# qq456cvb/CanonicalVoting

Hardware: AMD Instinct MI355X
Metric: scenes/sec (80k-pt synthetic scans) (higher is better)
Workload: dtype f32

## Files before the change

### canonicalvoting_amd/csrc/cv_common.h

```cpp
#pragma once
#include <hip/hip_runtime.h>

#include <cstdarg>
#include <cstdint>
#include <cstdio>

#include "cv_hip.h"

void cv_set_error(const char* fmt, ...);

#define CV_HIP_CHECK(expr)                                                                  \
    do {                                                                                    \
        hipError_t e_ = (expr);                                                             \
        if (e_ != hipSuccess) {                                                             \
            cv_set_error("%s failed: %s (%s:%d)", #expr, hipGetErrorString(e_), __FILE__,   \
                         __LINE__);                                                         \
            return CV_EHIP;                                                                 \
        }                                                                                   \
    } while (0)

#define CV_LAUNCH_CHECK() CV_HIP_CHECK(hipGetLastError())

#define CV_REQUIRE(cond, code, ...)     \
    do {                                \
        if (!(cond)) {                  \
            cv_set_error(__VA_ARGS__);  \
            return (code);              \
        }                               \
    } while (0)

__host__ __device__ static inline size_t cv_align_up(size_t v, size_t a) { return (v + a - 1) / a * a; }

struct CvCarver {
    char* base;
    size_t off = 0;
    explicit CvCarver(void* p) : base(static_cast<char*>(p)) {}
    template <typename T>
    T* take(size_t count) {
        off = cv_align_up(off, 256);
        T* r = reinterpret_cast<T*>(base + off);
        off += count * sizeof(T);
        return r;
    }
};

struct CvMapJob {
    const int32_t* out_coords; long long n_out;
    const unsigned long long* keys; const int32_t* vals; long long cap;
    int k, ts;
    int32_t* nbr;
    const int32_t* compose;
    const unsigned* bitmap;
    const int32_t* bbox;
    int up;
    int32_t* nbr3;
    int32_t* mask_words;
};
constexpr int CV_MAX_MAP_JOBS = 12;
int cv_sp_kernel_maps_batch(const CvMapJob* jobs, int n_jobs, void* stream);
constexpr long long CV_BITMAP_WORDS = 1ll << 20;
int cv_sp_occupancy_bitmap(const int32_t* d_coords, long long n, const int32_t* d_bbox, unsigned* d_bits, void* stream,
                           bool pre_cleared = false);

int cv_sp_build_levels_zero(int32_t* const* d_coords, unsigned long long* const* d_keys, int32_t* const* d_vals,
                            long long n, long long cap, int num_levels, int32_t* d_counts, int32_t* h_counts, void* d_ws,
                            size_t ws_bytes, int32_t* d_zero, long long n_zero, int32_t* d_set_one, void* stream,
                            uint32_t* d_bits = nullptr);

struct CvUpJob { const int32_t* nbr_down; long long n_coarse; int32_t* up; };
int cv_sp_up_maps_batch(const CvUpJob* jobs, int n_jobs, void* stream);

struct CvPermJob {
    const int32_t* nbr; long long n; int K, groups; int32_t* perm; int with_map;
    const int32_t* mask_words;
};
constexpr int CV_MAX_PERM_JOBS = 8;
int cv_hv_minmax_async_ex(const float* d_points, int64_t n, float* h_minmax6, void* d_ws, size_t ws_bytes, int32_t* d_zero_word,
                          int32_t* d_fill7f, void* stream);
int cv_decode_f32_ev(float* d_grid_obj, const float* d_grid_rot, const float* d_grid_scale, const int dims[3],
                     const float h_corner3[3], float res, const float* d_points, const float* d_xyz, const float* d_prob,
                     const int32_t* d_class, int64_t n, const cv_decode_params* params, int mutate_grid, void* d_ws, size_t ws_bytes,
                     int* h_n_cand, int64_t* h_cand_idx, int32_t* h_verdict, int* h_n_boxes, float* h_boxes, float* h_scores,
                     int32_t* h_classes, int* h_truncated, void* stream, void* ev_done);
int cv_decode_cat_f32_ev(float* d_grid_obj, const float* d_grid_rot, const float* d_grid_scale, const int dims[3],
                         const float h_corner3[3], float res, const float* d_points, const float* d_xyz, const float* d_prob,
                         const int32_t* d_class, int64_t n, int num_cats, const cv_decode_params* params, int mutate_grid,
                         void* d_ws, size_t ws_bytes, int* h_n_cand, int64_t* h_cand_idx, int32_t* h_verdict, int* h_n_boxes,
                         float* h_boxes, float* h_scores, int32_t* h_classes, int* h_truncated, void* stream, void* ev_done);
int cv_sp_sort_rows_ex(const int32_t* d_coords, long long n, int32_t* d_sorted, int32_t* d_perm, int32_t* d_inv, void* d_ws,
                       size_t ws_bytes, bool single_batch, void* stream, bool bounds_prefilled = false);
int cv_sp_scene_plan_ex(const int32_t* d_input, long long n, int32_t* d_perm, int32_t* d_inv, int32_t* const* d_coords,
                        unsigned long long* const* d_keys, int32_t* const* d_vals, long long cap, int32_t* d_counts,
                        int32_t* h_counts, int stem_k, int mask_groups, long long masked_min_rows,
                        int32_t* d_arena, size_t arena_words, cv_scene_maps* offsets, void* d_sort_ws, size_t sort_ws_bytes,
                        void* d_levels_ws, size_t levels_ws_bytes, bool single_batch, void* stream,
                        bool bounds_prefilled = false);
int cv_sp_mask_perms_batch(const CvPermJob* jobs, int n_jobs, void* d_ws, size_t ws_bytes, void* stream,
                           bool pre_zeroed = false);
```

### canonicalvoting_amd/csrc/hv_decode.hip

```cpp
#include "cv_common.h"

#include <cmath>
#include <cstring>
#include <mutex>
#include <vector>

namespace {

#ifndef DEC_PROF
#define DEC_PROF 0
#endif
constexpr int NCLS = 64;

struct Cand {
    long long idx;
    int c[3];
    int clo[3], chi[3];
    float cw[3];
    float cs, sn;
    float sc[3];
};

struct Stats {
    unsigned n_in, n_mask, pmax_bits, pad;
// ... 37 lines not shown
}

__global__ __launch_bounds__(256) void dec_compact(const float* __restrict__ g_obj,
                                                   const float* __restrict__ g_rot,
                                                   const float* __restrict__ g_scale, Geo geo,
                                                   int64_t G, float thresh, List L,
                                                   unsigned* __restrict__ list_n, CatStride ks) {
    const int kc = blockIdx.y;
    g_obj = g_obj + kc * ks.cells; g_rot = g_rot + kc * 2 * ks.cells; g_scale = g_scale + kc * 3 * ks.cells;
    L = cat_list(L, ks.ws, kc); list_n = cat_ws(list_n, ks.ws, kc);
    for (int64_t base = blockIdx.x * 256ll; base < G; base += (int64_t)gridDim.x * 256) {
        const int64_t i = base + threadIdx.x;
        float v = 0.f;
        bool hit = false;
        if (i < G) { v = g_obj[i]; hit = v >= thresh; }
        const uint64_t m = __ballot(hit);
        if (m == 0) continue;
        unsigned pos = 0;
        const int lane = threadIdx.x & 63;
        const int leader = __ffsll((unsigned long long)m) - 1;
        if (lane == leader) pos = atomicAdd(list_n, (unsigned)__popcll(m));
        pos = __shfl(pos, leader);
        if (hit) {
            const unsigned p = pos + lanes_below(m);
            const int id = (int)i;
            L.idx[p] = id;
            L.val[p] = v;
            const int z = id % geo.Z, y = (id / geo.Z) % geo.Y, x = id / (geo.Z * geo.Y);
            L.xy[p] = (unsigned)x | ((unsigned)y << 16);
            L.z[p] = z;
            const float r0 = g_rot[(int64_t)id * 2], r1 = g_rot[(int64_t)id * 2 + 1];
            const float rot = (float)atan2((double)r1, (double)r0);
            L.geo[0 * L.cap + p] = (float)cos((double)rot);
            L.geo[1 * L.cap + p] = (float)sin((double)rot);
            for (int k = 0; k < 3; ++k) L.geo[(2 + k) * L.cap + p] = g_scale[(int64_t)id * 3 + k];
        }
    }
}

__device__ __forceinline__ bool inv_coords(float d0, float d1, float d2, float c, float s,
                                           const float* sc, float& w0, float& w1, float& w2) {
    w0 = fmaf(d2, s, fmaf(d1, 0.f, d0 * c)) / sc[0];
    w1 = fmaf(d2, 0.f, fmaf(d1, 1.f, d0 * 0.f)) / sc[1];
    w2 = fmaf(d2, c, fmaf(d1, 0.f, d0 * (-s))) / sc[2];
    return -1 < w0 && w0 < 1 && -1 < w1 && w1 < 1 && -1 < w2 && w2 < 1;
}

__device__ __forceinline__ bool inside_box(float d0, float d1, float d2, float c, float s, const float* sc) {
    const float t0 = fmaf(d2, s, fmaf(d1, 0.f, d0 * c));
    const float t1 = fmaf(d2, 0.f, fmaf(d1, 1.f, d0 * 0.f));
    const float t2 = fmaf(d2, c, fmaf(d1, 0.f, d0 * (-s)));
    return fabsf(t0) < fabsf(sc[0]) && fabsf(t1) < fabsf(sc[1]) && fabsf(t2) < fabsf(sc[2]);
}

__device__ __forceinline__ void box_corners(float cs, float sn, const float* sc, float* bb) {
    constexpr float kRawX[8] = {1, 1, -1, -1, 1, 1, -1, -1};
    constexpr float kRawY[8] = {1, 1, 1, 1, -1, -1, -1, -1};
    constexpr float kRawZ[8] = {1, -1, -1, 1, 1, -1, -1, 1};
    const float m00 = cs * sc[0], m02 = (-sn) * sc[2], m11 = sc[1], m20 = sn * sc[0], m22 = cs * sc[2];
#pragma unroll
    for (int q = 0; q < 8; ++q) {
        bb[q * 3 + 0] = m00 * kRawX[q] + m02 * kRawZ[q];
        bb[q * 3 + 1] = m11 * kRawY[q];
        bb[q * 3 + 2] = m20 * kRawX[q] + m22 * kRawZ[q];
    }
}

struct Best {
    float v;
    int id, pos;
};

__device__ __forceinline__ void take_better(Best& b, float v, int id, int pos) {
    if (v > b.v || (v == b.v && id < b.id)) { b.v = v; b.id = id; b.pos = pos; }
}

#ifndef DEC_SMALL_T
#define DEC_SMALL_T 512
#endif
constexpr int GREEDY_T = DEC_SMALL_T;
constexpr int GREEDY_W = GREEDY_T / 64;
constexpr int GREEDY_CAP = 4096;

template <int CTRL>
__device__ __forceinline__ int dpp_mov(int x) {
    return __builtin_amdgcn_update_dpp(x, x, CTRL, 0xf, 0xf, false);
}
__device__ __forceinline__ float wave_max_f32(float x) {
    x = fmaxf(x, __int_as_float(dpp_mov<0xB1>(__float_as_int(x))));
    x = fmaxf(x, __int_as_float(dpp_mov<0x4E>(__float_as_int(x))));
    x = fmaxf(x, __int_as_float(dpp_mov<0x124>(__float_as_int(x))));
    x = fmaxf(x, __int_as_float(dpp_mov<0x128>(__float_as_int(x))));
    const int xi = __float_as_int(x);
    const float a = __int_as_float(__builtin_amdgcn_readlane(xi, 0)), b = __int_as_float(__builtin_amdgcn_readlane(xi, 16)),
                c = __int_as_float(__builtin_amdgcn_readlane(xi, 32)), d = __int_as_float(__builtin_amdgcn_readlane(xi, 48));
    return fmaxf(fmaxf(a, b), fmaxf(c, d));
}
__device__ __forceinline__ int wave_min_i32(int x) {
    x = min(x, dpp_mov<0xB1>(x));
    x = min(x, dpp_mov<0x4E>(x));
    x = min(x, dpp_mov<0x124>(x));
    x = min(x, dpp_mov<0x128>(x));
    return min(min(__builtin_amdgcn_readlane(x, 0), __builtin_amdgcn_readlane(x, 16)),
               min(__builtin_amdgcn_readlane(x, 32), __builtin_amdgcn_readlane(x, 48)));
}

template <int MODE, int T>
__device__ __forceinline__ void dec_greedy(Geo geo, cv_decode_params prm, List L,
                                           const unsigned* __restrict__ list_n, Cand* __restrict__ cands,
                                           Stats* __restrict__ stats, int* __restrict__ n_cand_out) {
    constexpr bool IN_REG = MODE != 0, IN_LDS = MODE == 1;
    constexpr int GREEDY_E = (MODE == 1 ? GREEDY_CAP / T : 16);
    constexpr int CAP = IN_LDS ? GREEDY_E * T : 1;
    constexpr int GREEDY_T = T, GREEDY_W = T / 64;
    __shared__ unsigned l_xy[CAP];
    __shared__ int l_z[CAP];
    __shared__ float l_geo[5][CAP];
    __shared__ float s_val[2][GREEDY_W];
    __shared__ int s_idx[2][GREEDY_W], s_pos[2][GREEDY_W];
    const int n = (int)*list_n;
    float r_val[GREEDY_E];
    unsigned r_xy[GREEDY_E], dead = 0;
    int r_z[GREEDY_E], r_id[GREEDY_E];
    if (IN_REG) {
#pragma unroll
        for (int j = 0; j < GREEDY_E; ++j) {
            const int k = (int)threadIdx.x + j * GREEDY_T;
            const bool ok = k < n;
            r_val[j] = ok ? L.val[k] : 0.f;
            r_xy[j] = ok ? L.xy[k] : 0u;
            r_z[j] = ok ? L.z[k] : 0;
            r_id[j] = ((int)(r_xy[j] & 0xffffu) * geo.Y + (int)(r_xy[j] >> 16)) * geo.Z + r_z[j];
            dead |= ok ? 0u : (1u << j);
            if (ok && IN_LDS) {
                l_xy[k] = r_xy[j];
                l_z[k] = r_z[j];
                for (int q = 0; q < 5; ++q) l_geo[q][k] = L.geo[q * L.cap + k];
            }
        }
        __syncthreads();
    }
    const int wave = threadIdx.x >> 6;
    const float inv_res = 1.0f / geo.res;
    const int e = prm.elimination, hp = e + (prm.elim_hi_plus1 ? 1 : 0);
    bool have_cur = false;
    int cx = 0, cy = 0, cz = 0, clo0 = 0, clo1 = 0, clo2 = 0, chi0 = 0, chi1 = 0, chi2 = 0;
    int rlo0 = 0, rlo1 = 0, rlo2 = 0;
    unsigned rsp0 = 0, rsp1 = 0, rsp2 = 0;
    float ccs = 0.f, csn = 0.f, csc[3] = {1.f, 1.f, 1.f};
    auto flat_id = [&](int pos) {
        const unsigned xy = L.xy[pos];
        const int z = L.z[pos];
        return ((int)(xy & 0xffffu) * geo.Y + (int)(xy >> 16)) * geo.Z + z;
    };
    int it = 0;
    bool truncated = false;
    for (;; ++it) {
        float bv = -1.f;
        int bpos = -1, bid = 0x7fffffff;
        if constexpr (IN_REG) {
            if (have_cur) {
                unsigned near = 0;
#pragma unroll
                for (int j = 0; j < GREEDY_E; ++j) {
                    const int x = (int)(r_xy[j] & 0xffffu), y = (int)(r_xy[j] >> 16), z = r_z[j];
                    const bool in = (unsigned)(x - rlo0) <= rsp0 && (unsigned)(y - rlo1) <= rsp1 &&
                                    (unsigned)(z - rlo2) <= rsp2;
                    near |= in ? (1u << j) : 0u;
                }
                near &= ~dead;
// ... 730 lines not shown
```

### canonicalvoting_amd/csrc/sparse_conv.hip

```cpp
#include "cv_common.h"

#include <atomic>
#include <cstring>
#include <type_traits>
#include <utility>

#include "sparse_conv_common.h"

using namespace cvsc;

namespace {

template <int NB, bool VEC>
__global__ __launch_bounds__(THREADS) void conv_rows(ConvArgs a) {
    __shared__ float A_s[KC][A_LD];
    __shared__ float B_s[KC][NB * 32];
    __shared__ int nbr_s[TM];
    __shared__ int rows_s[TM];
    __shared__ __attribute__((aligned(16))) float ep_s[4][32][EP_LD];
    const int tid = threadIdx.x, lane = tid & 63, wave = tid >> 6;
    const int n0 = blockIdx.y * (NB * 32);

    if (tid < TM) {
        const long long tile_id = a.row_perm ? (long long)gridDim.x - 1 - blockIdx.x : blockIdx.x;
// ... 383 lines not shown
                             : make_float4(0.f, 0.f, 0.f, 0.f);
        }
        const unsigned short* slab = second ? a.wp6_2 + (long long)c * P * a.cout * 32
                                            : a.wp6 + (long long)(j * nch + c) * P * a.cout * 32;
#pragma unroll
        for (int i = 0; i < B_PER; ++i) {
            const int f = tid + i * THREADS;
            if (f < B_U4) {
                const int p = f / (NB * 32 * 4), rem = f - p * (NB * 32 * 4);
                const int col = rem >> 2, ch = rem & 3;
                rb[i] = (n0 + col < a.cout)
                            ? *reinterpret_cast<const uint4*>(slab + ((long long)p * a.cout + n0 + col) * 32 + ch * 8)
                            : make_uint4(0u, 0u, 0u, 0u);
            }
        }
    };
    auto stage = [&](unsigned char* Bb) {
#pragma unroll
        for (int i = 0; i < 4; ++i) {
            const int r = a_row + 8 * i;
            unsigned h0 = 0, m0 = 0, l0 = 0, h1 = 0, m1 = 0, l1 = 0;
            unsigned char* dst = A_h + r * 64 + ((((a_col >> 3) ^ ((r >> 2) & 3))) << 4) + ((a_col & 7) << 1);
            if constexpr (P == 1) {
                *reinterpret_cast<uint2*>(dst) = make_uint2(cvt_pk_bf16(ra[i].x, ra[i].y), cvt_pk_bf16(ra[i].z, ra[i].w));
            } else if constexpr (P == 3) {
                split3(ra[i].x, ra[i].y, h0, m0, l0);
                split3(ra[i].z, ra[i].w, h1, m1, l1);
                *reinterpret_cast<uint2*>(dst) = make_uint2(h0, h1);
                *reinterpret_cast<uint2*>(dst + TM * 64) = make_uint2(m0, m1);
                *reinterpret_cast<uint2*>(dst + 2 * TM * 64) = make_uint2(l0, l1);
            } else {
                in_max = fmaxf(fmaxf(in_max, fmaxf(fabsf(ra[i].x), fabsf(ra[i].y))), fmaxf(fabsf(ra[i].z), fabsf(ra[i].w)));
                split2h(ra[i].x, ra[i].y, h0, l0);
                split2h(ra[i].z, ra[i].w, h1, l1);
                *reinterpret_cast<uint2*>(dst) = make_uint2(h0, h1);
                *reinterpret_cast<uint2*>(dst + TM * 64) = make_uint2(l0, l1);
            }
        }
#pragma unroll
        for (int i = 0; i < B_PER; ++i) {
            const int f = tid + i * THREADS;
            if (f < B_U4) {
                const int p = f / (NB * 32 * 4), rem = f - p * (NB * 32 * 4);
                const int col = rem >> 2, ch = rem & 3;
                *reinterpret_cast<uint4*>(Bb + (p * NB * 32 + col) * 64 + ((ch ^ ((col >> 2) & 3)) << 4)) = rb[i];
            }
        }
    };
    int j = j_first, c = c_first, buf = 0;
    if (njl > 0) skip_dead(j, c); else j = j_last + 1;
    if (j > j_last) { j = j_second; c = blockIdx.z; if (c >= nch2) j = j_done; }
    if (j < j_done) load(j, c);
#pragma unroll 1
    while (j < j_done) {
        unsigned char* Bb = B_h + buf * B_BYTES;
        stage(Bb);
        __syncthreads();
        const bool wave_live = __any(nbr_all[j - j_first][wave * 32 + l31] >= 0);
        advance(j, c);
        if (j < j_done) load(j, c);
        if (wave_live) compute(Bb);
        buf ^= 1;
    }
    __syncthreads();
    if constexpr (P == 2) {
        if (in_max > 65000.f && a.range_flag) *a.range_flag = 1;
        const float k = a.acc_scale;
#pragma unroll
        for (int nb = 0; nb < NB; ++nb)
#pragma unroll
            for (int r = 0; r < 16; ++r) acc[nb][r] *= k;
    }
    float (*ep)[EP_LD] = reinterpret_cast<float (*)[EP_LD]>(sm + wave * 32 * EP_LD * 4);
    if (a.wide) {
#pragma unroll
        for (int nb = 0; nb < NB; ++nb) epilogue_store_wide(a, acc[nb], rows_s + wave * 32, n0 + nb * 32, lane, ep);
    } else {
#pragma unroll
        for (int nb = 0; nb < NB; ++nb)
            epilogue_store(a, acc[nb], rows_s + wave * 32, n0 + nb * 32 + (lane & 31), lane);
    }
}

constexpr int HL_MAX_UNITS = 512;
constexpr int hl_blocks(int NB) { return NB <= 3 ? 4 : 2; }
template <int NB>
__global__ __attribute__((amdgpu_waves_per_eu(hl_blocks(NB), 8)))
__launch_bounds__(THREADS, hl_blocks(NB)) void conv_hl(ConvArgs a) {
    constexpr int NS = 2, NW = THREADS / 64;
    constexpr int B_BYTES = 2 * NB * 32 * 64, EP_BYTES = NW * 32 * EP_LD * 4;
    constexpr int SM_BYTES = NS * B_BYTES > EP_BYTES ? NS * B_BYTES : EP_BYTES;
    __shared__ __attribute__((aligned(16))) unsigned char sm[SM_BYTES];
    __shared__ int rows_s[TM];
    __shared__ int nbr_all[WP_NPRE + 1][TM];
    __shared__ unsigned wave_mask[NW];
    __shared__ unsigned short units_s[HL_MAX_UNITS + 4];
    const int tid = threadIdx.x, lane = tid & 63, wave = tid >> 6;
    const int n0 = blockIdx.y * (NB * 32);
    const long long tile_id = xcd_tile(a);
    if (tile_id * TM >= a.n_out) return;
    const int half = lane >> 5, l31 = lane & 31;
    const int nj = a.j_end - a.j_begin;
    const int nch = a.cin / KC;
    int u_lo, u_hi;
    if (a.perm_per_split) {
        u_lo = (int)((long long)nj * blockIdx.z / a.splits) * nch;
        u_hi = (int)((long long)nj * (blockIdx.z + 1) / a.splits) * nch;
    } else {
        u_lo = (int)((long long)nj * nch * blockIdx.z / a.splits);
        u_hi = (int)((long long)nj * nch * (blockIdx.z + 1) / a.splits);
    }
    const int j_first = a.j_begin + u_lo / nch, j_last = a.j_begin + (u_hi - 1) / nch;
    const int njl = u_hi > u_lo ? j_last - j_first + 1 : 0;
    const int nch2 = a.in2 ? a.cin2 / KC : 0;

    const int* perm = a.row_perm ? a.row_perm + (a.perm_per_split ? (long long)blockIdx.z * a.n_out : 0) : nullptr;
    if (tid < TM) {
        const long long t = tile_id * TM + tid;
        const int row = t < a.n_out ? (perm ? perm[t] : (int)t) : -1;
        rows_s[tid] = row;
        if (a.in2) nbr_all[njl][tid] = row;
    }
    {
        unsigned m = 0u;
        const int jg0 = a.j_begin + (int)((long long)nj * blockIdx.z / a.splits);
        for (int e = tid; e < njl * TM; e += THREADS) {
            const int jj = e / TM, t = e - jj * TM;
            const long long pos = tile_id * TM + t;
            int v = -1;
            if (pos < a.n_out) {
                if (a.nbr_perm) {
                    v = a.nbr_perm[((long long)blockIdx.z * a.n_out + pos) * a.nbr_perm_w + (j_first + jj - jg0)];
                } else {
                    const int row = perm ? perm[pos] : (int)pos;
                    v = a.nbr ? a.nbr[(long long)row * a.K + j_first + jj] : row;
                }
            }
            nbr_all[jj][t] = v;
            if (v >= 0) m |= 1u << jj;
        }
#pragma unroll
        for (int off = 32; off > 0; off >>= 1) m |= __shfl_xor(m, off);
        if (lane == 0) wave_mask[wave] = m;
    }
    __syncthreads();
    unsigned lm = 0u;
#pragma unroll
    for (int w = 0; w < NW; ++w) lm |= wave_mask[w];
    if (wave == 0) {
        const int n_first = u_hi - u_lo, n_second = nch2 > (int)blockIdx.z ? (nch2 - (int)blockIdx.z + a.splits - 1) / a.splits : 0;
        int cnt = 0;
        for (int base = 0; base < n_first + n_second; base += 64) {
            const int e = base + lane;
            int code = -1;
            if (e < n_first) {
                const int u = u_lo + e, q = u / nch;
                const int jj = a.j_begin + q - j_first;
                if ((lm >> jj) & 1u) code = (jj << 8) | (u - q * nch);
            } else if (e < n_first + n_second) {
                code = (njl << 8) | ((int)blockIdx.z + (e - n_first) * a.splits);
            }
            const unsigned long long bal = __ballot(code >= 0);
            if (code >= 0) units_s[cnt + __popcll(bal & ((1ull << lane) - 1ull))] = (unsigned short)code;
            cnt += __popcll(bal);
        }
        if (lane == 0) units_s[HL_MAX_UNITS] = (unsigned short)cnt;
    }
    __syncthreads();
    const int n_units = __builtin_amdgcn_readfirstlane((int)units_s[HL_MAX_UNITS]);
    if (n_units == 0 && a.gvalid) return;

    f32x16 acc[NB];
#pragma unroll
    for (int nb = 0; nb < NB; ++nb)
#pragma unroll
        for (int r = 0; r < 16; ++r) acc[nb][r] = 0.f;

    constexpr int B_U4 = 2 * NB * 32 * 4;
    constexpr int B_PER = (B_U4 + THREADS - 1) / THREADS;
    int b_src[B_PER], b_dst[B_PER];
#pragma unroll
    for (int i = 0; i < B_PER; ++i) {
        const int f = tid + i * THREADS;
        const int p = f / (NB * 32 * 4), rem = f - p * (NB * 32 * 4);
        const int col = rem >> 2, ch = rem & 3;
        b_src[i] = (f < B_U4 && n0 + col < a.cout) ? (p * a.cout + n0 + col) * 32 + ch * 8 : -1;
        b_dst[i] = f < B_U4 ? (p * NB * 32 + col) * 64 + ((ch ^ ((col >> 2) & 3)) << 4) : -1;
    }
    const unsigned slab_words = 2u * (unsigned)a.cout * 32u;
    const int my_row = wave * 32 + l31;
    const unsigned in_row_bytes = (unsigned)a.in_ld * 4u, in2_row_bytes = (unsigned)a.in2_ld * 4u;
    const unsigned char* const in_b = reinterpret_cast<const unsigned char*>(a.in);
    const unsigned char* const in2_b = reinterpret_cast<const unsigned char*>(a.in2);

    uint4 ra[NS][4], rb[NS][B_PER];
    bool live[NS];
#pragma unroll
    for (int q = 0; q < NS; ++q) live[q] = false;
    auto load = [&](auto S, int k) {
        constexpr int sl = decltype(S)::value;
        const int code = __builtin_amdgcn_readfirstlane((int)units_s[k]);
        const int jj = code >> 8, c = code & 255;
        const bool second = jj == njl;
        const int src = nbr_all[jj][my_row];
        live[sl] = __any(src >= 0);
        if (src >= 0) {
            const unsigned off = (unsigned)src * (second ? in2_row_bytes : in_row_bytes) + (unsigned)(c * 128 + half * 16);
            const unsigned char* p = (second ? in2_b : in_b) + off;
            ra[sl][0] = *reinterpret_cast<const uint4*>(p);
            ra[sl][1] = *reinterpret_cast<const uint4*>(p + 32);
            ra[sl][2] = *reinterpret_cast<const uint4*>(p + 64);
            ra[sl][3] = *reinterpret_cast<const uint4*>(p + 96);
        } else {
#pragma unroll
            for (int q = 0; q < 4; ++q) ra[sl][q] = make_uint4(0u, 0u, 0u, 0u);
        }
        const unsigned short* slab = second ? a.wp6_2 + (size_t)c * slab_words
                                            : a.wp6 + (size_t)((j_first + jj) * nch + c) * slab_words;
#pragma unroll
        for (int i = 0; i < B_PER; ++i)
            rb[sl][i] = b_src[i] >= 0 ? *reinterpret_cast<const uint4*>(slab + b_src[i]) : make_uint4(0u, 0u, 0u, 0u);
    };
    auto stage_b = [&](auto S, int toff) {
        constexpr int sl = decltype(S)::value;
#pragma unroll
        for (int i = 0; i < B_PER; ++i)
            if (b_dst[i] >= 0) *reinterpret_cast<uint4*>(sm + toff + b_dst[i]) = rb[sl][i];
    };
    const int b_rd = l31 * 64;
    const int bswz = (l31 >> 2) & 3;
    auto compute = [&](auto S, int toff) {
        constexpr int sl = decltype(S)::value;
        const unsigned char* Bb = sm + toff + b_rd;
        uint4 (&fa)[4] = ra[sl];
#pragma unroll
        for (int ks = 0; ks < 2; ++ks) {
            const int piece = ((2 * ks + half) ^ bswz) << 4;
            const f16x8 a0 = __builtin_bit_cast(f16x8, fa[ks]), a1 = __builtin_bit_cast(f16x8, fa[2 + ks]);
#pragma unroll
            for (int nb = 0; nb < NB; ++nb) {
                const f16x8 b0 = *reinterpret_cast<const f16x8*>(Bb + nb * 32 * 64 + piece);
                const f16x8 b1 = *reinterpret_cast<const f16x8*>(Bb + (NB * 32 + nb * 32) * 64 + piece);
                acc[nb] = __builtin_amdgcn_mfma_f32_32x32x16_f16(a0, b1, acc[nb], 0, 0, 0);
                acc[nb] = __builtin_amdgcn_mfma_f32_32x32x16_f16(a1, b0, acc[nb], 0, 0, 0);
                acc[nb] = __builtin_amdgcn_mfma_f32_32x32x16_f16(a0, b0, acc[nb], 0, 0, 0);
                if constexpr (NB >= 3) asm volatile("" ::: "memory");
            }
        }
    };
    typedef std::integral_constant<int, 0> S0;
    typedef std::integral_constant<int, 1> S1;
    if (n_units > 0) load(S0{}, 0);
    if (n_units > 1) load(S1{}, 1);
    if (n_units > 0) stage_b(S0{}, 0);
    auto step = [&](auto S, auto SN, int k) {
        constexpr int sl = decltype(S)::value;
        __syncthreads();
        if (k + 1 < n_units) stage_b(SN, decltype(SN)::value * B_BYTES);
        if (live[sl]) compute(S, sl * B_BYTES);
        if (k + 2 < n_units) load(S, k + 2);
    };
#pragma unroll 1
    for (int k = 0; k < n_units; k += 2) {
        step(S0{}, S1{}, k);
        if (k + 1 >= n_units) break;
        step(S1{}, S0{}, k + 1);
    }
    __syncthreads();
    {
        const float sc = a.acc_scale_dev ? a.acc_scale * *a.acc_scale_dev : a.acc_scale;
#pragma unroll
        for (int nb = 0; nb < NB; ++nb)
#pragma unroll
            for (int r = 0; r < 16; ++r) acc[nb][r] *= sc;
    }
    float (*ep)[EP_LD] = reinterpret_cast<float (*)[EP_LD]>(sm + wave * 32 * EP_LD * 4);
#pragma unroll
    for (int nb = 0; nb < NB; ++nb) epilogue_store_wide(a, acc[nb], rows_s + wave * 32, n0 + nb * 32, lane, ep);
    if (a.splits > 1 && a.tickets) {
        __shared__ int last_flag;
        asm volatile("s_waitcnt vmcnt(0)" ::: "memory");
        __syncthreads();
        int* ticket = a.tickets + tile_id * gridDim.y + blockIdx.y;
        if (tid == 0) {
            const int old = __hip_atomic_fetch_add(ticket, 1, __ATOMIC_RELAXED, __HIP_MEMORY_SCOPE_AGENT);
            last_flag = old == a.splits - 1;
            if (last_flag) __builtin_amdgcn_fence(__ATOMIC_ACQUIRE, "agent");
        }
        __syncthreads();
        if (!last_flag) return;
        if (tid == 0) *ticket = 0;
        const long long plane = a.n_out * (long long)a.cout;
#pragma unroll
        for (int nb = 0; nb < NB; ++nb) {
            const int col = n0 + nb * 32 + (lane & 7) * 4;
            if (col >= a.cout) continue;
#pragma unroll
            for (int it = 0; it < 4; ++it) {
                const int row = rows_s[wave * 32 + (lane >> 3) + 8 * it];
                if (row < 0) continue;
                const float* p = a.partial + (long long)row * a.cout + col;
                float4 sq[4];
#pragma unroll
                for (int q = 0; q < 4; ++q) sq[q] = make_float4(0.f, 0.f, 0.f, 0.f);
                for (int k0 = 0; k0 < a.splits; k0 += 4) {
#pragma unroll
                    for (int q = 0; q < 4; ++q)
                        if (k0 + q < a.splits) {
                            const float4 v = *reinterpret_cast<const float4*>(p + (long long)(k0 + q) * plane);
                            sq[q].x += v.x; sq[q].y += v.y; sq[q].z += v.z; sq[q].w += v.w;
                        }
                }
                const float4 x = make_float4(sq[0].x + sq[1].x + sq[2].x + sq[3].x, sq[0].y + sq[1].y + sq[2].y + sq[3].y,
                                             sq[0].z + sq[1].z + sq[2].z + sq[3].z, sq[0].w + sq[1].w + sq[2].w + sq[3].w);
                epilogue_apply4(a, row, col, x);
            }
        }
    }
}

constexpr int hd_lds_bytes(int NB, int NW, int NSTG) {
    return NSTG * (NW * 4096 + 2 * NB * 32 * 64) + NW * 32 * 4 + (WP_NPRE + 1) * NW * 32 * 4 + NW * 4 + (HL_MAX_UNITS + 4) * 2;
}
constexpr int hd_blocks(int NB, int NW, int NSTG) {
    const int b = (160 * 1024) / hd_lds_bytes(NB, NW, NSTG);
    return b * NW > 32 ? 32 / NW : (b < 1 ? 1 : b);
}
template <int NB, int NW, int NSTG>
__global__ __launch_bounds__(NW * 64, (hd_blocks(NB, NW, NSTG) * NW + 3) / 4) void conv_hd(ConvArgs a) {
    static_assert(NSTG == 2 || NSTG == 3, "two or three ring stages");
    constexpr int TMv = NW * 32, THv = NW * 64;
    constexpr int A_BYTES = NW * 4096, B_BYTES = 2 * NB * 32 * 64, STAGE = A_BYTES + B_BYTES;
    constexpr int B_INSTR = B_BYTES / 1024;
    constexpr int B_PER_WAVE = (B_INSTR + NW - 1) / NW;
    constexpr int EP_BYTES = NW * 32 * EP_LD * 4;
    static_assert(EP_BYTES <= NSTG * STAGE, "the epilogue tile aliases the ring");
    constexpr int OFF_ROWS = NSTG * STAGE, OFF_NBR = OFF_ROWS + TMv * 4, OFF_MASK = OFF_NBR + (WP_NPRE + 1) * TMv * 4,
                  OFF_UNITS = OFF_MASK + NW * 4,
                  LDS_TOTAL = OFF_UNITS + (HL_MAX_UNITS + 4) * 2;
    static_assert(LDS_TOTAL == hd_lds_bytes(NB, NW, NSTG) && LDS_TOTAL <= 160 * 1024, "LDS budget");
    __shared__ __attribute__((aligned(1024))) unsigned char lds[LDS_TOTAL];
    unsigned char* const sm = lds;
// ... 2043 lines not shown
```

### profiles/microbench/gather_rate.hip

```cpp
#include <hip/hip_runtime.h>
#include <cstdio>
#include <cstdint>
#include <vector>

#define CK(x) do { hipError_t e_ = (x); if (e_ != hipSuccess) { printf("%s: %s\n", #x, hipGetErrorString(e_)); return 1; } } while (0)

template <int MODE, int DEPTH>
__global__ __launch_bounds__(256, 4) void gather(const unsigned char* __restrict__ buf, const int* __restrict__ idx,
                                                  int units, int row_bytes, int chunks, unsigned* __restrict__ out) {
    const int lane = threadIdx.x & 63;
    const int wave = (blockIdx.x * 256 + threadIdx.x) >> 6;
    const int* my = idx + (size_t)wave * units * 32;
    uint4 acc = make_uint4(0, 0, 0, 0);
    uint4 r[DEPTH][4];
    auto issue = [&](int s, int u) {
        const int c = u % chunks;
        if (MODE == 0) {
            const int row = my[u * 32 + (lane & 31)];
            const unsigned char* p = buf + (size_t)row * row_bytes + c * 128 + (lane >> 5) * 16;
#pragma unroll
            for (int q = 0; q < 4; ++q) r[s][q] = *reinterpret_cast<const uint4*>(p + 32 * q);
        } else if (MODE == 1) {
#pragma unroll
            for (int q = 0; q < 4; ++q) {
                const int row = my[u * 32 + (lane >> 3) + 8 * q];
                r[s][q] = *reinterpret_cast<const uint4*>(buf + (size_t)row * row_bytes + c * 128 + (lane & 7) * 16);
            }
        } else if (MODE == 2) {
#pragma unroll
            for (int q = 0; q < 4; ++q) {
                const int row = my[u * 32 + (lane & 15) + 16 * (q & 1)];
                r[s][q] = *reinterpret_cast<const uint4*>(buf + (size_t)row * row_bytes + c * 128 + (q >> 1) * 64 + (lane >> 4) * 16);
            }
        } else {
            const int row = my[u * 32 + (lane >> 1)];
            const unsigned char* p = buf + (size_t)row * row_bytes + c * 128 + (lane & 1) * 16;
#pragma unroll
            for (int q = 0; q < 4; ++q) r[s][q] = *reinterpret_cast<const uint4*>(p + 32 * q);
        }
    };
    auto eat = [&](int s) {
#pragma unroll
        for (int q = 0; q < 4; ++q) { acc.x ^= r[s][q].x; acc.y ^= r[s][q].y; acc.z ^= r[s][q].z; acc.w ^= r[s][q].w; }
    };
#pragma unroll
    for (int s = 0; s < DEPTH - 1; ++s) issue(s, s);
#pragma unroll 1
    for (int u = 0; u < units; u += DEPTH) {
#pragma unroll
        for (int s = 0; s < DEPTH; ++s) {
            const int nxt = u + s + DEPTH - 1;
            if (nxt < units) issue((s + DEPTH - 1) % DEPTH, nxt);
            if (u + s < units) eat(s);
        }
    }
    if ((acc.x ^ acc.y ^ acc.z ^ acc.w) == 0x12345u) out[wave] = acc.x;
}

template <int MODE, int DEPTH>
static int run(const char* name, const unsigned char* buf, const int* idx, int units, int row_bytes, int chunks, unsigned* out,
               int wgs, double clock_ghz, int cus) {
    hipEvent_t e0, e1;
    CK(hipEventCreate(&e0)); CK(hipEventCreate(&e1));
    for (int w = 0; w < 2; ++w) gather<MODE, DEPTH><<<wgs, 256>>>(buf, idx, units, row_bytes, chunks, out);
    CK(hipEventRecord(e0));
    const int reps = 5;
    for (int w = 0; w < reps; ++w) gather<MODE, DEPTH><<<wgs, 256>>>(buf, idx, units, row_bytes, chunks, out);
    CK(hipEventRecord(e1));
    CK(hipEventSynchronize(e1));
    float ms; CK(hipEventElapsedTime(&ms, e0, e1));
    ms /= reps;
    const double bytes = (double)wgs * 4 * units * 4096.0;
    printf("  %-34s depth %d: %8.1f us  %7.2f TB/s  %6.2f B/clk/CU\n", name, DEPTH, ms * 1e3, bytes / ms / 1e9,
           bytes / (ms * 1e-3) / (clock_ghz * 1e9) / cus);
    return 0;
}

int main() {
    hipDeviceProp_t prop; CK(hipGetDeviceProperties(&prop, 0));
    const int cus = prop.multiProcessorCount;
    const double ghz = prop.clockRate / 1e6;
    printf("%s: %d CUs, %.2f GHz\n", prop.name, cus, ghz);
    const int row_bytes = 384, chunks = 3, units = 96;
    const int wgs = cus * 4, waves = wgs * 4;
    const int max_rows = 80000;
    unsigned char* buf; int* idx; unsigned* out;
    CK(hipMalloc(&buf, (size_t)max_rows * row_bytes)); CK(hipMemset(buf, 1, (size_t)max_rows * row_bytes));
    CK(hipMalloc(&idx, (size_t)waves * units * 32 * 4)); CK(hipMalloc(&out, waves * 4));
    std::vector<int> h((size_t)waves * units * 32);
    struct Case { int rows; int per_xcd; const char* what; };
    const Case cases[] = {{1024, 0, "0.4 MB working set (fits the 32 KB L1s poorly, the L2 well)"},
                          {4096, 0, "1.5 MB working set (every XCD's L2 holds all of it)"},
                          {10000, 0, "3.75 MB working set (just inside a 4 MB L2)"},
                          {80000, 0, "30 MB working set (Infinity Cache)"},
                          {80000, 1, "30 MB, each XCD draws from its own eighth (3.75 MB per L2)"},
                          {40000, 1, "15 MB, each XCD draws from its own eighth (1.9 MB per L2)"}};
    for (const Case& cs : cases) {
        uint32_t s = 12345u;
        for (int w = 0; w < waves; ++w) {
            const int wg = w / 4, xcd = wg % 8;
            const int lo = cs.per_xcd ? xcd * (cs.rows / 8) : 0, span = cs.per_xcd ? cs.rows / 8 : cs.rows;
            for (int u = 0; u < units; ++u)
                for (int r = 0; r < 32; ++r) {
                    s = s * 1664525u + 1013904223u;
                    const int row = lo + (int)((s >> 8) % (unsigned)span);
                    h[((size_t)w * units + u) * 32 + r] = (u % chunks) ? h[((size_t)w * units + u - (u % chunks)) * 32 + r] : row;
                }
        }
        CK(hipMemcpy(idx, h.data(), h.size() * 4, hipMemcpyHostToDevice));
        printf("%s\n", cs.what);
        if (run<0, 2>("MFMA 32x32 layout (lane = row)", buf, idx, units, row_bytes, chunks, out, wgs, ghz, cus)) return 1;
        if (run<0, 3>("MFMA 32x32 layout (lane = row)", buf, idx, units, row_bytes, chunks, out, wgs, ghz, cus)) return 1;
        if (run<2, 2>("MFMA 16x16 layout (4 lanes / 64 B)", buf, idx, units, row_bytes, chunks, out, wgs, ghz, cus)) return 1;
        if (run<1, 2>("line-coalesced (8 lanes per chunk)", buf, idx, units, row_bytes, chunks, out, wgs, ghz, cus)) return 1;
        if (run<1, 3>("line-coalesced (8 lanes per chunk)", buf, idx, units, row_bytes, chunks, out, wgs, ghz, cus)) return 1;
    }
    return 0;
}
```

Baseline: 626.2.

## Gather conv input rows in quad-coalesced form and transpose via DPP

The sparse conv hl kernel now has each lane quad load the same 128-byte chunk slice from four neighbour rows, so four lanes together cover a contiguous 128 bytes of one row. Previously each lane loaded four 16-byte pieces at 32-byte strides from its own row. Cross-lane DPP exchanges inside each quad then restore the lane-per-row register layout the MFMA compute expects. The intent is better-coalesced gather loads from cache. The cost is extra DPP moves and selects per unit, and a liveness test changed to a per-quad row check. Profiling scripts and a microbenchmark with a correctness check for the transposition are also added.

```diff
diff --git a/canonicalvoting_amd/csrc/cv_common.h b/canonicalvoting_amd/csrc/cv_common.h
--- a/canonicalvoting_amd/csrc/cv_common.h
+++ b/canonicalvoting_amd/csrc/cv_common.h
@@ -28,6 +28,11 @@
             return (code);              \
         }                               \
     } while (0)
+
+template <int CTRL>
+__device__ __forceinline__ int dpp_mov(int x) {
+    return __builtin_amdgcn_update_dpp(x, x, CTRL, 0xf, 0xf, false);
+}
 
 __host__ __device__ static inline size_t cv_align_up(size_t v, size_t a) { return (v + a - 1) / a * a; }
 
diff --git a/canonicalvoting_amd/csrc/hv_decode.hip b/canonicalvoting_amd/csrc/hv_decode.hip
--- a/canonicalvoting_amd/csrc/hv_decode.hip
+++ b/canonicalvoting_amd/csrc/hv_decode.hip
@@ -143,10 +143,6 @@
 constexpr int GREEDY_W = GREEDY_T / 64;
 constexpr int GREEDY_CAP = 4096;
 
-template <int CTRL>
-__device__ __forceinline__ int dpp_mov(int x) {
-    return __builtin_amdgcn_update_dpp(x, x, CTRL, 0xf, 0xf, false);
-}
 __device__ __forceinline__ float wave_max_f32(float x) {
     x = fmaxf(x, __int_as_float(dpp_mov<0xB1>(__float_as_int(x))));
     x = fmaxf(x, __int_as_float(dpp_mov<0x4E>(__float_as_int(x))));
diff --git a/canonicalvoting_amd/csrc/sparse_conv.hip b/canonicalvoting_amd/csrc/sparse_conv.hip
--- a/canonicalvoting_amd/csrc/sparse_conv.hip
+++ b/canonicalvoting_amd/csrc/sparse_conv.hip
@@ -489,6 +489,20 @@
     }
 }
 
+
+template <int CTRL>
+__device__ __forceinline__ void hl_quad_xchg(uint4& a, uint4& b, bool hi) {
+    const auto one = [&](unsigned& x, unsigned& y) {
+        const unsigned t = (unsigned)dpp_mov<CTRL>((int)(hi ? x : y));
+        x = hi ? t : x;
+        y = hi ? y : t;
+    };
+    one(a.x, b.x); one(a.y, b.y); one(a.z, b.z); one(a.w, b.w);
+}
+__device__ __forceinline__ void hl_quad_transpose(uint4 (&r)[4], bool b0, bool b1) {
+    hl_quad_xchg<0xB1>(r[0], r[1], b0); hl_quad_xchg<0xB1>(r[2], r[3], b0);
+    hl_quad_xchg<0x4E>(r[0], r[2], b1); hl_quad_xchg<0x4E>(r[1], r[3], b1);
+}
 constexpr int HL_MAX_UNITS = 512;
 constexpr int hl_blocks(int NB) { return NB <= 3 ? 4 : 2; }
 template <int NB>
@@ -499,7 +513,7 @@
     constexpr int SM_BYTES = NS * B_BYTES > EP_BYTES ? NS * B_BYTES : EP_BYTES;
     __shared__ __attribute__((aligned(16))) unsigned char sm[SM_BYTES];
     __shared__ int rows_s[TM];
-    __shared__ int nbr_all[WP_NPRE + 1][TM];
+    __shared__ __attribute__((aligned(16))) int nbr_all[WP_NPRE + 1][TM];
     __shared__ unsigned wave_mask[NW];
     __shared__ unsigned short units_s[HL_MAX_UNITS + 4];
     const int tid = threadIdx.x, lane = tid & 63, wave = tid >> 6;
@@ -595,7 +609,9 @@
         b_dst[i] = f < B_U4 ? (p * NB * 32 + col) * 64 + ((ch ^ ((col >> 2) & 3)) << 4) : -1;
     }
     const unsigned slab_words = 2u * (unsigned)a.cout * 32u;
-    const int my_row = wave * 32 + l31;
+    const int quad_row = wave * 32 + (l31 & ~3);
+    const unsigned quad_off = (unsigned)((lane & 3) * 32 + half * 16);
+    const bool q_b0 = lane & 1, q_b1 = lane & 2;
     const unsigned in_row_bytes = (unsigned)a.in_ld * 4u, in2_row_bytes = (unsigned)a.in2_ld * 4u;
     const unsigned char* const in_b = reinterpret_cast<const unsigned char*>(a.in);
     const unsigned char* const in2_b = reinterpret_cast<const unsigned char*>(a.in2);
@@ -609,19 +625,19 @@
         const int code = __builtin_amdgcn_readfirstlane((int)units_s[k]);
         const int jj = code >> 8, c = code & 255;
         const bool second = jj == njl;
-        const int src = nbr_all[jj][my_row];
-        live[sl] = __any(src >= 0);
-        if (src >= 0) {
-            const unsigned off = (unsigned)src * (second ? in2_row_bytes : in_row_bytes) + (unsigned)(c * 128 + half * 16);
-            const unsigned char* p = (second ? in2_b : in_b) + off;
-            ra[sl][0] = *reinterpret_cast<const uint4*>(p);
-            ra[sl][1] = *reinterpret_cast<const uint4*>(p + 32);
-            ra[sl][2] = *reinterpret_cast<const uint4*>(p + 64);
-            ra[sl][3] = *reinterpret_cast<const uint4*>(p + 96);
-        } else {
-#pragma unroll
-            for (int q = 0; q < 4; ++q) ra[sl][q] = make_uint4(0u, 0u, 0u, 0u);
-        }
+        const int4 src = *reinterpret_cast<const int4*>(&nbr_all[jj][quad_row]);
+        live[sl] = __any((src.x & src.y & src.z & src.w) >= 0);
+        const unsigned row_bytes = second ? in2_row_bytes : in_row_bytes, c_off = (unsigned)(c * 128) + quad_off;
+        const unsigned char* const base = second ? in2_b : in_b;
+        const auto row_piece = [&](int r) {
+            uint4 v = make_uint4(0u, 0u, 0u, 0u);
+            if (r >= 0) v = *reinterpret_cast<const uint4*>(base + ((unsigned)r * row_bytes + c_off));
+            return v;
+        };
+        ra[sl][0] = row_piece(src.x);
+        ra[sl][1] = row_piece(src.y);
+        ra[sl][2] = row_piece(src.z);
+        ra[sl][3] = row_piece(src.w);
         const unsigned short* slab = second ? a.wp6_2 + (size_t)c * slab_words
                                             : a.wp6 + (size_t)((j_first + jj) * nch + c) * slab_words;
 #pragma unroll
@@ -664,7 +680,10 @@
         constexpr int sl = decltype(S)::value;
         __syncthreads();
         if (k + 1 < n_units) stage_b(SN, decltype(SN)::value * B_BYTES);
-        if (live[sl]) compute(S, sl * B_BYTES);
+        if (live[sl]) {
+            hl_quad_transpose(ra[sl], q_b0, q_b1);
+            compute(S, sl * B_BYTES);
+        }
         if (k + 2 < n_units) load(S, k + 2);
     };
 #pragma unroll 1
diff --git a/profiles/hl_gather_summary.py b/profiles/hl_gather_summary.py
--- /dev/null
+++ b/profiles/hl_gather_summary.py
@@ -0,0 +1,76 @@
+import collections
+import csv
+import gzip
+import json
+import os
+import sys
+
+sys.path.insert(0, os.path.dirname(os.path.abspath(__file__)))
+from in_flight_summary import family, find
+
+BUCKETS = ((64, "< 64"), (256, "64-255"), (1024, "256-1023"), (1 << 30, ">= 1024"))
+
+
+def bucket(w):
+    return next(name for lim, name in BUCKETS if w < lim)
+
+
+def main():
+    tdir, bench_json = sys.argv[1:3]
+    bench = json.loads(open(bench_json).read().strip().splitlines()[-1])
+    steps = bench["steps"]
+    tfile = tdir if tdir.endswith((".gz", ".csv")) else find(tdir, "kernel_trace.csv")
+    rows = list(csv.DictReader(gzip.open(tfile, "rt") if tfile.endswith(".gz") else open(tfile)))
+    def wgs(r):
+        try:
+            g = [int(r[k]) for k in ("Grid_Size_X", "Grid_Size_Y", "Grid_Size_Z")]
+            w = [max(1, int(r[k])) for k in ("Workgroup_Size_X", "Workgroup_Size_Y", "Workgroup_Size_Z")]
+            return max(1, (g[0] // w[0]) * max(1, g[1] // w[1]) * max(1, g[2] // w[2]))
+        except (KeyError, ValueError):
+            return int(r.get("Grid_Size", 0)) // max(1, int(r.get("Workgroup_Size", 1)))
+    ev = sorted((int(r["Start_Timestamp"]), int(r["End_Timestamp"]), r["Kernel_Name"], wgs(r)) for r in rows)
+    heads = [e for e in ev if family(e[2]) == "head"]
+    iso = 2 * 4 + max(min(steps, 48), 24)
+    assert len(heads) >= steps + iso, (len(heads), steps, iso)
+    t_lo, t_hi = heads[-(steps + iso) + 20][0], heads[-(iso + 20) - 1][1]
+    a_lo = heads[-(iso - 8)][0]
+    print("trace run: %.1f scenes/s under the tracer over %d steps" % (bench["value"], steps))
+    for label, lo, hi in (("seven in flight", t_lo, t_hi), ("alone", a_lo, ev[-1][1] + 1)):
+        scenes = len([h for h in heads if lo < h[1] <= hi])
+        dur, cnt = collections.defaultdict(float), collections.Counter()
+        per = collections.defaultdict(list)
+        for s, e, n, w in ev:
+            if s >= lo and e <= hi:
+                f = family(n)
+                dur[f] += (e - s) * 1e-6
+                cnt[f] += 1
+                if f == "conv_hl":
+                    per[bucket(w)].append((e - s) * 1e-3)
+        print("\n%s: %d scenes" % (label, scenes))
+        print("  %-14s %10s %18s" % ("family", "launches", "kernel ms / scene"))
+        for f in ("conv_hl", "conv_hd", "conv_finish", "conv_stem"):
+            print("  %-14s %10.1f %18.3f" % (f, cnt[f] / scenes, dur[f] / scenes))
+        print("  %-14s %10.1f %18.3f" % ("all kernels", sum(cnt.values()) / scenes, sum(dur.values()) / scenes))
+        print("  conv_hl by launch size (workgroups): launches / scene, mean us per launch, us / scene")
+        for _, name in BUCKETS:
+            v = per.get(name, [])
+            if v:
+                print("    %-9s %6.1f %9.2f %10.1f" % (name, len(v) / scenes, sum(v) / len(v), sum(v) / scenes))
+    for d in sys.argv[3:]:
+        rows = list(csv.DictReader(open(find(d, "counter_collection.csv"))))
+        per = collections.defaultdict(lambda: collections.defaultdict(float))
+        disp = collections.defaultdict(set)
+        for r in rows:
+            f = family(r["Kernel_Name"])
+            per[f][r["Counter_Name"]] += float(r["Counter_Value"])
+            disp[f].add(r["Dispatch_Id"])
+        scenes = max(1, len(disp["head"]))
+        names = sorted({c for f in per for c in per[f]})
+        print("\ncounters per scene (%d scenes, kernels serialised by the profiler): %s" % (scenes, d))
+        print("  %-14s %9s " % ("family", "launches") + " ".join("%18s" % c[-18:] for c in names))
+        for f in ("conv_hl", "conv_hd", "conv_finish"):
+            print("  %-14s %9.1f " % (f, len(disp[f]) / scenes) + " ".join("%18.5g" % (per[f].get(c, 0.0) / scenes) for c in names))
+
+
+if __name__ == "__main__":
+    main()
diff --git a/profiles/microbench/gather_rate.hip b/profiles/microbench/gather_rate.hip
--- a/profiles/microbench/gather_rate.hip
+++ b/profiles/microbench/gather_rate.hip
@@ -5,7 +5,86 @@
 
 #define CK(x) do { hipError_t e_ = (x); if (e_ != hipSuccess) { printf("%s: %s\n", #x, hipGetErrorString(e_)); return 1; } } while (0)
 
-template <int MODE, int DEPTH>
+template <int CTRL>
+__device__ __forceinline__ unsigned dpp_mov(unsigned x) {
+    return (unsigned)__builtin_amdgcn_update_dpp((int)x, (int)x, CTRL, 0xf, 0xf, false);
+}
+template <class MOVE>
+__device__ __forceinline__ void xchg(unsigned& a, unsigned& b, bool hi, MOVE mv) {
+    const unsigned t = mv(hi ? a : b);
+    a = hi ? t : a;
+    b = hi ? b : t;
+}
+template <class MOVE>
+__device__ __forceinline__ void xchg4(uint4& a, uint4& b, bool hi, MOVE mv) {
+    xchg(a.x, b.x, hi, mv); xchg(a.y, b.y, hi, mv); xchg(a.z, b.z, hi, mv); xchg(a.w, b.w, hi, mv);
+}
+__device__ __forceinline__ unsigned flip05(unsigned x, bool b0, bool b5) {
+    const unsigned t = dpp_mov<0xB1>(x);
+    const auto sw = __builtin_amdgcn_permlane32_swap(t, t, false, false);
+    const unsigned u = b5 ? sw[0] : sw[1];
+    return b0 != b5 ? u : x;
+}
+template <int MODE>
+__device__ __forceinline__ void transpose(uint4 (&r)[4], int lane) {
+    const auto x1 = [](unsigned v) { return dpp_mov<0xB1>(v); };
+    const auto x2 = [](unsigned v) { return dpp_mov<0x4E>(v); };
+    const auto x4 = [](unsigned v) { return dpp_mov<0x141>(dpp_mov<0x1B>(v)); };
+    if (MODE == 4) {
+        xchg4(r[0], r[1], lane & 1, x1); xchg4(r[2], r[3], lane & 1, x1);
+        xchg4(r[0], r[2], lane & 2, x2); xchg4(r[1], r[3], lane & 2, x2);
+    } else if (MODE == 5) {
+        xchg4(r[0], r[1], lane & 2, x2); xchg4(r[2], r[3], lane & 2, x2);
+        xchg4(r[0], r[2], lane & 4, x4); xchg4(r[1], r[3], lane & 4, x4);
+        const bool b0 = lane & 1, b5 = lane & 32;
+#pragma unroll
+        for (int q = 0; q < 4; ++q) {
+            r[q].x = flip05(r[q].x, b0, b5); r[q].y = flip05(r[q].y, b0, b5);
+            r[q].z = flip05(r[q].z, b0, b5); r[q].w = flip05(r[q].w, b0, b5);
+        }
+    }
+}
+template <int MODE>
+__device__ __forceinline__ void issue_unit(uint4 (&r)[4], const unsigned char* __restrict__ buf, const int* my, int u, int c,
+                                           int row_bytes, int lane) {
+    if (MODE == 4) {
+        const int4 rows = *reinterpret_cast<const int4*>(my + u * 32 + ((lane >> 2) & 7) * 4);
+        const unsigned o = c * 128 + (lane & 3) * 32 + (lane >> 5) * 16;
+        r[0] = *reinterpret_cast<const uint4*>(buf + (size_t)rows.x * row_bytes + o);
+        r[1] = *reinterpret_cast<const uint4*>(buf + (size_t)rows.y * row_bytes + o);
+        r[2] = *reinterpret_cast<const uint4*>(buf + (size_t)rows.z * row_bytes + o);
+        r[3] = *reinterpret_cast<const uint4*>(buf + (size_t)rows.w * row_bytes + o);
+    } else {
+        const int g = lane >> 3;
+#pragma unroll
+        for (int q = 0; q < 4; ++q) {
+            const int row = my[u * 32 + ((g >> 1) & 1) * 16 + (g & 1) * 8 + q * 2 + (g >> 2)];
+            r[q] = *reinterpret_cast<const uint4*>(buf + (size_t)row * row_bytes + c * 128 + (lane & 7) * 16);
+        }
+    }
+}
+template <int MODE>
+__global__ __launch_bounds__(64) void check(const unsigned char* __restrict__ buf, const int* __restrict__ idx, int row_bytes,
+                                            int chunks, int units, unsigned* __restrict__ bad) {
+    const int lane = threadIdx.x;
+    unsigned n = 0;
+    for (int u = 0; u < units; ++u) {
+        uint4 r[4];
+        issue_unit<MODE>(r, buf, idx, u, u % chunks, row_bytes, lane);
+        transpose<MODE>(r, lane);
+        const unsigned base = (unsigned)idx[u * 32 + (lane & 31)] * 128u + (u % chunks) * 32 + (lane >> 5) * 4;
+#pragma unroll
+        for (int k = 0; k < 4; ++k)
+            n += (r[k].x != base + 8 * k) + (r[k].y != base + 8 * k + 1) + (r[k].z != base + 8 * k + 2) + (r[k].w != base + 8 * k + 3);
+    }
+    if (n) atomicAdd(bad, n);
+}
+__global__ void fill_pattern(unsigned* __restrict__ buf, size_t rows, int row_dwords) {
+    for (size_t i = blockIdx.x * (size_t)blockDim.x + threadIdx.x; i < rows * row_dwords; i += (size_t)gridDim.x * blockDim.x)
+        buf[i] = (unsigned)(i / row_dwords) * 128u + (unsigned)(i % row_dwords);
+}
+
+template <int MODE, int DEPTH, bool XP = false>
 __global__ __launch_bounds__(256, 4) void gather(const unsigned char* __restrict__ buf, const int* __restrict__ idx,
                                                   int units, int row_bytes, int chunks, unsigned* __restrict__ out) {
     const int lane = threadIdx.x & 63;
@@ -32,14 +111,17 @@
                 const int row = my[u * 32 + (lane & 15) + 16 * (q & 1)];
                 r[s][q] = *reinterpret_cast<const uint4*>(buf + (size_t)row * row_bytes + c * 128 + (q >> 1) * 64 + (lane >> 4) * 16);
             }
-        } else {
+        } else if (MODE == 3) {
             const int row = my[u * 32 + (lane >> 1)];
             const unsigned char* p = buf + (size_t)row * row_bytes + c * 128 + (lane & 1) * 16;
 #pragma unroll
             for (int q = 0; q < 4; ++q) r[s][q] = *reinterpret_cast<const uint4*>(p + 32 * q);
+        } else {
+            issue_unit<MODE>(r[s], buf, my, u, c, row_bytes, lane);
         }
     };
     auto eat = [&](int s) {
+        if (XP) transpose<MODE>(r[s], lane);
 #pragma unroll
         for (int q = 0; q < 4; ++q) { acc.x ^= r[s][q].x; acc.y ^= r[s][q].y; acc.z ^= r[s][q].z; acc.w ^= r[s][q].w; }
     };
@@ -57,15 +139,15 @@
     if ((acc.x ^ acc.y ^ acc.z ^ acc.w) == 0x12345u) out[wave] = acc.x;
 }
 
-template <int MODE, int DEPTH>
+template <int MODE, int DEPTH, bool XP = false>
 static int run(const char* name, const unsigned char* buf, const int* idx, int units, int row_bytes, int chunks, unsigned* out,
                int wgs, double clock_ghz, int cus) {
     hipEvent_t e0, e1;
     CK(hipEventCreate(&e0)); CK(hipEventCreate(&e1));
-    for (int w = 0; w < 2; ++w) gather<MODE, DEPTH><<<wgs, 256>>>(buf, idx, units, row_bytes, chunks, out);
+    for (int w = 0; w < 2; ++w) gather<MODE, DEPTH, XP><<<wgs, 256>>>(buf, idx, units, row_bytes, chunks, out);
     CK(hipEventRecord(e0));
     const int reps = 5;
-    for (int w = 0; w < reps; ++w) gather<MODE, DEPTH><<<wgs, 256>>>(buf, idx, units, row_bytes, chunks, out);
+    for (int w = 0; w < reps; ++w) gather<MODE, DEPTH, XP><<<wgs, 256>>>(buf, idx, units, row_bytes, chunks, out);
     CK(hipEventRecord(e1));
     CK(hipEventSynchronize(e1));
     float ms; CK(hipEventElapsedTime(&ms, e0, e1));
@@ -85,7 +167,7 @@
     const int wgs = cus * 4, waves = wgs * 4;
     const int max_rows = 80000;
     unsigned char* buf; int* idx; unsigned* out;
-    CK(hipMalloc(&buf, (size_t)max_rows * row_bytes)); CK(hipMemset(buf, 1, (size_t)max_rows * row_bytes));
+    CK(hipMalloc(&buf, (size_t)max_rows * row_bytes)); fill_pattern<<<1024, 256>>>(reinterpret_cast<unsigned*>(buf), max_rows, row_bytes / 4);
     CK(hipMalloc(&idx, (size_t)waves * units * 32 * 4)); CK(hipMalloc(&out, waves * 4));
     std::vector<int> h((size_t)waves * units * 32);
     struct Case { int rows; int per_xcd; const char* what; };
@@ -95,6 +177,7 @@
                           {80000, 0, "30 MB working set (Infinity Cache)"},
                           {80000, 1, "30 MB, each XCD draws from its own eighth (3.75 MB per L2)"},
                           {40000, 1, "15 MB, each XCD draws from its own eighth (1.9 MB per L2)"}};
+    bool checked = false;
     for (const Case& cs : cases) {
         uint32_t s = 12345u;
         for (int w = 0; w < waves; ++w) {
@@ -108,12 +191,29 @@
                 }
         }
         CK(hipMemcpy(idx, h.data(), h.size() * 4, hipMemcpyHostToDevice));
+        if (!checked) {
+            unsigned* bad; unsigned hb[2];
+            CK(hipMalloc(&bad, 8)); CK(hipMemset(bad, 0, 8));
+            check<4><<<1, 64>>>(buf, idx, row_bytes, chunks, units, bad);
+            check<5><<<1, 64>>>(buf, idx, row_bytes, chunks, units, bad + 1);
+            CK(hipMemcpy(hb, bad, 8, hipMemcpyDeviceToHost));
+            printf("transposition check against the lane = row registers: quad form %u, eight-lane form %u mismatching dwords\n", hb[0], hb[1]);
+            if (hb[0] | hb[1]) return 1;
+            checked = true;
+        }
         printf("%s\n", cs.what);
         if (run<0, 2>("MFMA 32x32 layout (lane = row)", buf, idx, units, row_bytes, chunks, out, wgs, ghz, cus)) return 1;
         if (run<0, 3>("MFMA 32x32 layout (lane = row)", buf, idx, units, row_bytes, chunks, out, wgs, ghz, cus)) return 1;
         if (run<2, 2>("MFMA 16x16 layout (4 lanes / 64 B)", buf, idx, units, row_bytes, chunks, out, wgs, ghz, cus)) return 1;
         if (run<1, 2>("line-coalesced (8 lanes per chunk)", buf, idx, units, row_bytes, chunks, out, wgs, ghz, cus)) return 1;
         if (run<1, 3>("line-coalesced (8 lanes per chunk)", buf, idx, units, row_bytes, chunks, out, wgs, ghz, cus)) return 1;
+        if (run<3, 2>("two adjacent lanes per row", buf, idx, units, row_bytes, chunks, out, wgs, ghz, cus)) return 1;
+        if (run<4, 2>("quad form (Q), loads only", buf, idx, units, row_bytes, chunks, out, wgs, ghz, cus)) return 1;
+        if (run<4, 2, true>("quad form (Q) + transposition", buf, idx, units, row_bytes, chunks, out, wgs, ghz, cus)) return 1;
+        if (run<4, 3, true>("quad form (Q) + transposition", buf, idx, units, row_bytes, chunks, out, wgs, ghz, cus)) return 1;
+        if (run<5, 2>("eight-lane form (E), loads only", buf, idx, units, row_bytes, chunks, out, wgs, ghz, cus)) return 1;
+        if (run<5, 2, true>("eight-lane form (E) + transposition", buf, idx, units, row_bytes, chunks, out, wgs, ghz, cus)) return 1;
+        if (run<5, 3, true>("eight-lane form (E) + transposition", buf, idx, units, row_bytes, chunks, out, wgs, ghz, cus)) return 1;
     }
     return 0;
 }
```

Measured after the change: 624.7. No clear change (-0.2%).
